# livesense-inc/fanlin-rs

Measured on AMD Instinct MI355X. Metric: images/sec whole-node (1080p→300×200 resize+encode); p50 per-image ms, higher is better.
Workload: dtype u8 (exact, as f16 subnormals) x the reference's f32 weights as three f16 terms -> f32 sums (vertical, v_mfma_f32_16x16x32_f16); 24-bit fixed-point intermediate (2^-14 steps, three i8 planes) x 24-bit fixed-point weights (2^-24 steps, three i8 digits), eight of the nine digit products -> exact i32 (h

## Files before the change

### fanlin-rs_amd/csrc/fl_jpeg_dev.h

```cpp
#pragma once
#include <hip/hip_runtime.h>
#include <stdint.h>

#include "fl_jpeg.h"
#include "fl_jpeg_tables.h"
#include "fl_pixel.h"
#include "fl_types.h"

namespace fl {

namespace {


constexpr int32_t F_0_298 = 2446, F_0_390 = 3196, F_0_541 = 4433, F_0_765 = 6270, F_0_899 = 7373, F_1_175 = 9633, F_1_501 = 12299,
                  F_1_847 = 15137, F_1_961 = 16069, F_2_053 = 16819, F_2_562 = 20995, F_3_072 = 25172;

struct Mat8 { int32_t a[8][8]; };

constexpr void fdct_linear(const int32_t in[8], int32_t out[8])
{
    int32_t t0 = in[0] + in[7], t1 = in[1] + in[6], t2 = in[2] + in[5], t3 = in[3] + in[4];
    const int32_t t10 = t0 + t3, t11 = t1 + t2;
    int32_t t12 = t0 - t3, t13 = t1 - t2;
    t0 = in[0] - in[7]; t1 = in[1] - in[6]; t2 = in[2] - in[5]; t3 = in[3] - in[4];
    out[0] = t10 + t11;
    out[4] = t10 - t11;
    int32_t z1 = (t12 + t13) * F_0_541;
    out[2] = z1 + t12 * F_0_765;
    out[6] = z1 - t13 * F_1_847;
    t12 = t0 + t2;
    t13 = t1 + t3;
    z1 = (t12 + t13) * F_1_175;
    t12 = t12 * (-F_0_390) + z1;
    t13 = t13 * (-F_1_961) + z1;
    z1 = (t0 + t3) * (-F_0_899);
    out[1] = t0 * F_1_501 + z1 + t12;
    out[7] = t3 * F_0_298 + z1 + t13;
    z1 = (t1 + t2) * (-F_2_562);
    out[3] = t1 * F_3_072 + z1 + t13;
    out[5] = t2 * F_2_053 + z1 + t12;
}

constexpr Mat8 make_fdct_matrix()
{
    Mat8 m{};
    for (int j = 0; j < 8; ++j) {
        int32_t e[8] = {0, 0, 0, 0, 0, 0, 0, 0}, o[8] = {0, 0, 0, 0, 0, 0, 0, 0};
        e[j] = 1;
        fdct_linear(e, o);
        for (int k = 0; k < 8; ++k) m.a[k][j] = o[k];
    }
    return m;
}

__constant__ Mat8 kFdct = make_fdct_matrix();

constexpr bool fdct_matrix_fits_i16()
{
    const Mat8 m = make_fdct_matrix();
    for (int k = 0; k < 8; ++k)
        for (int j = 0; j < 8; ++j)
            if (m.a[k][j] > 32767 || m.a[k][j] < -32768) return false;
    return true;
}
static_assert(fdct_matrix_fits_i16(), "the passes use v_dot2_i32_i16: matrix entries must be 16-bit");

typedef short i16x2 __attribute__((ext_vector_type(2)));
__device__ __forceinline__ i16x2 as_i16x2(uint32_t v) { return __builtin_bit_cast(i16x2, v); }
__device__ __forceinline__ uint32_t pack_i16(int32_t lo, int32_t hi) { return ((uint32_t)lo & 0xffffu) | ((uint32_t)hi << 16); }
__device__ __forceinline__ int32_t dot8_i16(const uint32_t m[4], const uint4 v)
{
    int32_t p = __builtin_amdgcn_sdot2(as_i16x2(m[0]), as_i16x2(v.x), 0, false);
    p = __builtin_amdgcn_sdot2(as_i16x2(m[1]), as_i16x2(v.y), p, false);
    p = __builtin_amdgcn_sdot2(as_i16x2(m[2]), as_i16x2(v.z), p, false);
    return __builtin_amdgcn_sdot2(as_i16x2(m[3]), as_i16x2(v.w), p, false);
}

struct NaturalOrder { uint8_t n[64]; };
constexpr NaturalOrder make_natural()
{
    NaturalOrder t{};
    for (int k = 0; k < 64; ++k) t.n[k] = kUnzigzag[k];
    return t;
}
__constant__ NaturalOrder kNatural = make_natural();

struct HuffLut { uint32_t e[256]; };

constexpr HuffLut make_lut(const HuffSpec &s)
{
    HuffLut t{};
    uint32_t code = 0;
    int k = 0;
    for (int l = 1; l <= 16; ++l) {
        for (int i = 0; i < s.len[l - 1]; ++i, ++k) t.e[s.val[k]] = ((uint32_t)l << 16) | code++;
        code <<= 1;
    }
    return t;
}

struct HuffAll { HuffLut ac[2], dc[2]; };
constexpr HuffAll make_all() { return HuffAll{{make_lut(kAcLuma), make_lut(kAcChroma)}, {make_lut(kDcLuma), make_lut(kDcChroma)}}; }
__constant__ HuffAll kHuff = make_all();


template <int N>
__device__ __forceinline__ uint32_t dpp_row_shr(uint32_t v)
{
    return (uint32_t)__builtin_amdgcn_update_dpp(0, (int)v, 0x110 + N, 0xf, 0xf, false);
}

__device__ __forceinline__ uint32_t wave_inclusive_scan(uint32_t v, uint32_t lane)
{
    (void)lane;
    v += dpp_row_shr<1>(v);
    v += dpp_row_shr<2>(v);
    v += dpp_row_shr<4>(v);
    v += dpp_row_shr<8>(v);
    v += (uint32_t)__builtin_amdgcn_update_dpp(0, (int)v, 0x142, 0xa, 0xf, false);
    v += (uint32_t)__builtin_amdgcn_update_dpp(0, (int)v, 0x143, 0xc, 0xf, false);
    return v;
}

__device__ __forceinline__ void wave_lds_sync()
{
    __builtin_amdgcn_fence(__ATOMIC_SEQ_CST, "wavefront");
    __builtin_amdgcn_wave_barrier();
}

constexpr uint32_t kPackThreads = 512;
constexpr uint32_t kPackWaves = kPackThreads / 64;

__device__ __forceinline__ uint32_t wg_exclusive_scan(uint32_t v, uint32_t *s_w, uint32_t *total)
{
    const uint32_t lane = threadIdx.x & 63u, wave = threadIdx.x >> 6;
    const uint32_t inc = wave_inclusive_scan(v, lane);
    __syncthreads();
    if (lane == 63u) s_w[wave] = inc;
    __syncthreads();
    uint32_t base = 0, sum = 0;
#pragma unroll
    for (uint32_t i = 0; i < kPackWaves; ++i) { const uint32_t t = s_w[i]; if (i < wave) base += t; sum += t; }
    *total = sum;
    return base + inc - v;
}

__device__ __forceinline__ uint32_t coef_size(int32_t v)
{
    const uint32_t mag = (uint32_t)(v < 0 ? -v : v);
    return mag ? 32u - (uint32_t)__clz(mag) : 0u;
}


#ifndef FL_JPEG_BPW
#define FL_JPEG_BPW 16
#define FL_JPEG_WPG 2
#define FL_JPEG_PREFETCH 3
#endif
constexpr uint32_t kBlocksPerWave = FL_JPEG_BPW;
constexpr uint32_t kWavesPerWg = FL_JPEG_WPG;
constexpr uint32_t kPrefetch = FL_JPEG_PREFETCH;
static_assert(kBlocksPerWave == 32u || kBlocksPerWave == 16u, "the coding phase's lane mapping");
constexpr uint32_t kJpegThreads = 64u * kWavesPerWg;
constexpr uint32_t kBlocksPerWg = kWavesPerWg * kBlocksPerWave;
constexpr uint32_t kUnitsPerWave = 3u * kBlocksPerWave;

static_assert(63u * (16u + 10u) <= kAcWordsPerUnit * 32u, "a unit's AC code must fit its acbits slot");

struct WaveLds {
    int16_t coef[kUnitsPerWave][64];
    uint64_t nz[kUnitsPerWave];
    __attribute__((aligned(16))) int16_t smp[3][64];
    __attribute__((aligned(16))) int16_t p1[3][64];
};

__device__ __forceinline__ void stage_ac_luts(uint32_t *s_ac, const uint32_t *own = nullptr)
{
    if (own) for (uint32_t i = threadIdx.x; i < 512u; i += kJpegThreads) s_ac[i] = own[i];
    else for (uint32_t i = threadIdx.x; i < 512u; i += kJpegThreads) s_ac[i] = kHuff.ac[i >> 8].e[i & 255u];
    __syncthreads();
}

template <bool kRgba>
__device__ __forceinline__ uint32_t block_pixel(const JpegJob &jb, uint32_t brow, uint32_t bcol, uint32_t r, uint32_t c)
{
    uint32_t px = bcol * 8u + c, py = brow * 8u + r;
    px = px < jb.w ? px : jb.w - 1u;
    py = py < jb.h ? py : jb.h - 1u;
    if constexpr (kRgba) return ((const __attribute__((address_space(1))) uint32_t *)jb.src)[(size_t)py * jb.w + px];
    uint32_t pr, pg, pb, pa;
    load_rgba(jb.src + ((size_t)py * jb.w + px) * jb.c, jb.c, pr, pg, pb, pa);
    return pr | (pg << 8) | (pb << 16);
}

__device__ __forceinline__ void dct_quant_block(const uint32_t (&smp)[3], uint32_t nat, uint32_t r, uint32_t c, const uint32_t (&m1)[4],
                                                const uint32_t (&m2)[4], uint4 k1, const uint32_t (&q)[3], const uint32_t (&magic)[3],
                                                WaveLds &w, int32_t (&qv)[3])
{
#pragma unroll
    for (int k = 0; k < 3; ++k) w.smp[k][nat] = (int16_t)smp[k];
    wave_lds_sync();
#pragma unroll
    for (int k = 0; k < 3; ++k) {
        const int32_t p = dot8_i16(m1, *reinterpret_cast<const uint4 *>(w.smp[k] + r * 8));
        const int32_t v1 = ((p << k1.x) + (int32_t)k1.y) >> 11;
        w.p1[k][c * 8 + r] = (int16_t)v1;
    }
    wave_lds_sync();
#pragma unroll
    for (int k = 0; k < 3; ++k) {
        const int32_t p2 = dot8_i16(m2, *reinterpret_cast<const uint4 *>(w.p1[k] + c * 8));
        const int32_t d = (p2 + (int32_t)k1.z) >> k1.w;
        const int32_t sg = d >> 31;
        const uint32_t an = (uint32_t)((d ^ sg) - sg) >> 3;
        const uint32_t rq = __umulhi(2u * an + q[k], magic[k]);
        qv[k] = ((int32_t)rq ^ sg) - sg;
    }
}

typedef __attribute__((address_space(1))) uint32_t global_u32;
typedef uint32_t u32x4 __attribute__((ext_vector_type(4)));
typedef __attribute__((address_space(1))) u32x4 global_u32x4;
static_assert(sizeof(JpegUnit) == sizeof(u32x4) && kUnitAcWords == 3u, "a unit's record is one 16-byte access");

struct UnitBits {
    uint64_t acc;
    uint32_t pend, total, wi;
    global_u32 *out;
    uint32_t w0, w1, w2;
    __device__ __forceinline__ void word(uint32_t v)
    {
        w0 = wi == 0u ? v : w0;
        w1 = wi == 1u ? v : w1;
        w2 = wi == 2u ? v : w2;
        if (wi >= kUnitAcWords) out[wi] = v;
        ++wi;
    }
    __device__ __forceinline__ void put(uint32_t code, uint32_t len)
    {
        acc = (acc << len) | code;
        pend += len;
        total += len;
        if (pend >= 32u) { pend -= 32u; word((uint32_t)(acc >> pend)); }
    }
};

template <bool kRgba>
__device__ __forceinline__ void transform_blocks(const JpegJob &jb, const uint32_t *__restrict__ arena, uint32_t first, uint32_t count,
                                                 uint32_t lane, WaveLds &w)
{
    const uint32_t nat = kNatural.n[lane], r = nat >> 3, c = nat & 7u;
    uint32_t m1[4], m2[4];
#pragma unroll
    for (int j = 0; j < 4; ++j) {
        m1[j] = pack_i16(kFdct.a[c][2 * j], kFdct.a[c][2 * j + 1]);
        m2[j] = pack_i16(kFdct.a[r][2 * j], kFdct.a[r][2 * j + 1]);
    }
    const uint8_t *qt = reinterpret_cast<const uint8_t *>(arena + jb.tab_off) + 624;
    const uint32_t *mg = reinterpret_cast<const uint32_t *>(qt + 128);
    const uint32_t q[3] = {qt[nat], qt[64 + nat], qt[64 + nat]};
    const uint32_t magic[3] = {mg[nat], mg[64 + nat], mg[64 + nat]};
    const uint4 k1 = {(c == 0u || c == 4u) ? 13u : 0u, c == 0u ? (uint32_t)(-(8 * 128) * 8192) : (c == 4u ? 0u : 1u << 10),
                      (r == 0u || r == 4u) ? 2u : 1u << 14, (r == 0u || r == 4u) ? 2u : 15u};
    uint32_t brow = first / jb.bx, bcol = first - brow * jb.bx;
    uint32_t ahead[kPrefetch];
#pragma unroll
    for (uint32_t j = 0; j < kPrefetch; ++j) {
        ahead[j] = block_pixel<kRgba>(jb, brow, bcol, r, c);
        if (++bcol == jb.bx) { bcol = 0; ++brow; }
    }
    for (uint32_t i = 0; i < count; ++i) {
        const uint32_t rgb = kRgba ? ahead[0] & 0xffffffu : ahead[0];
#pragma unroll
        for (uint32_t j = 0; j + 1u < kPrefetch; ++j) ahead[j] = ahead[j + 1u];
        ahead[kPrefetch - 1u] = block_pixel<kRgba>(jb, brow, bcol, r, c);
        if (++bcol == jb.bx) { bcol = 0; ++brow; }
        uint32_t smp[3];
        jfif_px(rgb, smp[0], smp[1], smp[2]);
        const bool flat = __ballot(rgb != (uint32_t)__builtin_amdgcn_readfirstlane((int)rgb)) == 0ull;
        if (flat) {
            if (lane == 0u) {
#pragma unroll
                for (int k = 0; k < 3; ++k) {
                    const int32_t d = 64 * ((int32_t)smp[k] - 128);
                    const int32_t sg = d >> 31;
                    const uint32_t an = (uint32_t)((d ^ sg) - sg) >> 3;
                    const uint32_t rq = __umulhi(2u * an + q[k], magic[k]);
                    w.coef[i * 3u + k][0] = (int16_t)(((int32_t)rq ^ sg) - sg);
                    w.nz[i * 3u + k] = 0ull;
                }
            }
            continue;
        }
        int32_t qv[3];
        dct_quant_block(smp, nat, r, c, m1, m2, k1, q, magic, w, qv);
#pragma unroll
        for (int k = 0; k < 3; ++k) {
            w.coef[i * 3u + k][lane] = (int16_t)qv[k];
            const uint64_t nz = __ballot(qv[k] != 0) & ~1ull;
            if (lane == 0u) w.nz[i * 3u + k] = nz;
        }
    }
}

template <bool kOwn>
__device__ __forceinline__ void jpeg_code_units(const JpegJob *__restrict__ jobs, const uint32_t *__restrict__ arena, uint32_t job_base,
                                                const uint32_t *__restrict__ opt)
{
    __shared__ WaveLds s_w[kWavesPerWg];
    __shared__ uint32_t s_ac[512];
    const JpegJob jb = jobs[job_base + blockIdx.y];
    const uint32_t wave = threadIdx.x >> 6, lane = threadIdx.x & 63u;
    const uint32_t nblocks = jb.bx * jb.by;
    if (blockIdx.x * kBlocksPerWg >= nblocks) return;
    if constexpr (kOwn) stage_ac_luts(s_ac, opt + jb.opt_off + kJpegOptAcLut);
    else stage_ac_luts(s_ac);
    const uint32_t first = blockIdx.x * kBlocksPerWg + wave * kBlocksPerWave;
    if (first >= nblocks) return;
    const uint32_t count = min(kBlocksPerWave, nblocks - first);
    WaveLds &w = s_w[wave];

    if (jb.c == 4u && (reinterpret_cast<uintptr_t>(jb.src) & 3u) == 0u) transform_blocks<true>(jb, arena, first, count, lane, w);
    else transform_blocks<false>(jb, arena, first, count, lane, w);
    wave_lds_sync();

    uint32_t b, u, u_end;
    bool chroma;
    if constexpr (kBlocksPerWave == 32u) {
        b = lane & 31u;
        chroma = lane >= 32u;
        u = b * 3u + (chroma ? 1u : 0u);
        u_end = b * 3u + (chroma ? 3u : 1u);
    } else {
        b = lane & 15u;
        chroma = lane >= 16u;
        u = b * 3u + (lane >> 4);
        u_end = lane >= 48u ? u : u + 1u;
    }
    if (b >= count) return;
    const uint32_t *tab = s_ac + (chroma ? 256u : 0u);
    const uint32_t eob = tab[0], zrl = tab[0xF0];
    for (; u < u_end; ++u) {
        const uint32_t unit = first * 3u + u;
        const int16_t *cf = w.coef[u];
        uint64_t m = w.nz[u];
        UnitBits ub{0ull, 0u, 0u, 0u, (global_u32 *)jb.acbits + (size_t)unit * kAcWordsPerUnit, 0u, 0u, 0u};
        uint32_t prev = 0;
        uint32_t pos = (uint32_t)__builtin_ctzll(m | (1ull << 63));
        int32_t v = cf[pos];
        while (m) {
            const uint32_t cpos = pos;
            const int32_t cv = v;
            m &= m - 1ull;
            pos = (uint32_t)__builtin_ctzll(m | (1ull << 63));
            v = cf[pos];
            uint32_t run = cpos - prev - 1u;
            prev = cpos;
            while (run > 15u) { ub.put(zrl & 0xffffu, zrl >> 16); run -= 16u; }
            const uint32_t mag = (uint32_t)(cv < 0 ? -cv : cv);
            const uint32_t size = 32u - (uint32_t)__clz(mag);
            const uint32_t value = (uint32_t)(cv + (cv >> 31)) & ((1u << size) - 1u);
            const uint32_t e = tab[(run << 4) | size];
            ub.put(((e & 0xffffu) << size) | value, (e >> 16) + size);
        }
        if (prev != 63u) ub.put(eob & 0xffffu, eob >> 16);
        if (ub.pend) ub.word((uint32_t)(ub.acc << (32u - ub.pend)));
        const u32x4 rec = {((uint32_t)(uint16_t)cf[0]) | (ub.total << 16), ub.w0, ub.w1, ub.w2};
        ((global_u32x4 *)jb.units)[unit] = rec;
    }
}


constexpr uint32_t kDcCodes = 12;

constexpr uint32_t kWinWords = 8192;

__device__ __forceinline__ void win_or(uint32_t *win, uint32_t wbase, uint64_t g, uint32_t val)
{
    const uint64_t W = g >> 5;
    const uint32_t sh = (uint32_t)g & 31u;
    const uint32_t hi = val >> sh, lo = sh ? val << (32u - sh) : 0u;
    if (hi && W >= wbase && W < (uint64_t)wbase + kWinWords) atomicOr(&win[W - wbase], hi);
    if (lo && W + 1 >= wbase && W + 1 < (uint64_t)wbase + kWinWords) atomicOr(&win[W + 1 - wbase], lo);
}

__device__ __forceinline__ uint32_t dc_code(const uint32_t *s_dc, uint32_t u, uint32_t meta, uint32_t prev_meta, uint32_t *len)
{
    const int32_t dc = (int16_t)(meta & 0xffffu), prev = (int16_t)(prev_meta & 0xffffu);
    const int32_t diff = dc - prev;
    const uint32_t size = coef_size(diff);
    const uint32_t value = (uint32_t)(diff < 0 ? diff - 1 : diff) & ((1u << size) - 1u);
    const uint32_t e = s_dc[((u % 3u) ? kDcCodes : 0u) + size];
    *len = (e >> 16) + size;
    return (((e & 0xffffu) << size) | value) << (32u - *len);
}

struct PackUnit { u32x4 rec; uint32_t prev; };
__device__ __forceinline__ PackUnit load_pack_unit(const JpegJob &jb, uint32_t u, uint32_t u_end)
{
    const global_u32x4 *recs = (const global_u32x4 *)jb.units;
    const uint32_t uc = min(u, u_end - 1u);
    PackUnit p;
    p.rec = recs[uc];
    p.prev = ((const global_u32 *)(recs + (max(uc, 3u) - 3u)))[0];
    return p;
}
__device__ __forceinline__ PackUnit take_pack_unit(PackUnit p, uint32_t u, uint32_t u_end)
{
    if (u >= u_end) p.rec = u32x4{0u, 0u, 0u, 0u};
    if (u < 3u || u >= u_end) p.prev = 0u;
    return p;
}

#ifndef FL_JPEG_PACK_DEPTH
#define FL_JPEG_PACK_DEPTH 1
#endif
constexpr uint32_t kPackDepth = FL_JPEG_PACK_DEPTH;

template <bool kOwn>
__global__ __launch_bounds__(kPackThreads) void jpeg_pack_kernel(const JpegJob *__restrict__ jobs, const uint32_t *__restrict__ arena,
                                                                 uint32_t job_base, const uint32_t *__restrict__ opt)
{
    __shared__ uint32_t s_win[kWinWords];
    __shared__ uint32_t s_w[kPackWaves], s_carry, s_lo, s_hi, s_dc[2u * kDcCodes];
    const JpegJob jb = jobs[job_base + blockIdx.x];
    const uint32_t tid = threadIdx.x;
    const uint32_t nunits = jb.bx * jb.by * 3u;
    constexpr uint32_t T = kPackThreads;

    PackUnit ahead[kPackDepth];
#pragma unroll
    for (uint32_t j = 0; j < kPackDepth; ++j) ahead[j] = load_pack_unit(jb, j * T + tid, nunits);
    for (uint32_t i = tid; i < kWinWords; i += T) s_win[i] = 0u;
    const uint32_t *own = kOwn ? opt + jb.opt_off : nullptr;
    if constexpr (kOwn) { if (tid < 2u * kDcCodes) s_dc[tid] = own[kJpegOptDcLut + tid]; }
    else if (tid < 2u * kDcCodes) s_dc[tid] = kHuff.dc[tid / kDcCodes].e[tid % kDcCodes];
    if (tid == 0u) s_carry = 0u;
    __syncthreads();
    for (uint32_t base0 = 0; base0 < nunits; base0 += kPackDepth * T) {
#pragma unroll
        for (uint32_t j = 0; j < kPackDepth; ++j) {
            const uint32_t base = base0 + j * T;
            if (base >= nunits) break;
            const uint32_t u = base + tid;
            const PackUnit next = load_pack_unit(jb, u + kPackDepth * T, nunits);
            const PackUnit cur = take_pack_unit(ahead[j], u, nunits);
            ahead[j] = next;
            const uint32_t m = cur.rec.x;
            const uint32_t nw = ((m >> 16) + 31u) >> 5;
            uint32_t len = 0, dl = 0, dcw = 0;
            if (u < nunits) {
                dcw = dc_code(s_dc, u, m, cur.prev, &dl);
                len = dl + (m >> 16);
            }
            uint32_t chunk;
            const uint32_t ex = wg_exclusive_scan(len, s_w, &chunk);
            const uint32_t carry = s_carry;
            if (u < nunits) {
                const uint32_t off = carry + ex;
                ((global_u32 *)jb.unit_off)[u] = off;
                win_or(s_win, 0u, off, dcw);
                win_or(s_win, 0u, (uint64_t)off + dl, cur.rec.y);
                win_or(s_win, 0u, (uint64_t)off + dl + 32u, cur.rec.z);
                win_or(s_win, 0u, (uint64_t)off + dl + 64u, cur.rec.w);
                for (uint32_t w = kUnitAcWords; w < nw; ++w)
                    win_or(s_win, 0u, (uint64_t)off + dl + 32u * w, ((const global_u32 *)jb.acbits)[(size_t)u * kAcWordsPerUnit + w]);
            }
            __syncthreads();
            if (tid == 0u) s_carry = carry + chunk;
            __syncthreads();
        }
    }
    const uint32_t total_bits = s_carry;
    if (tid == 0u) jb.unit_off[nunits] = total_bits;
    __threadfence_block();
    __syncthreads();
    const uint32_t nbytes = (total_bits + 7u) >> 3, limit = jb.dst_cap;
    const uint8_t *hdr = reinterpret_cast<const uint8_t *>(kOwn ? own + kJpegOptHeader : arena + jb.tab_off);
    const uint32_t hdr_bytes = kOwn ? own[kJpegOptHdrLen] : kJpegHeaderBytes;
    for (uint32_t i = tid; i < hdr_bytes; i += T) if (i < limit) jb.dst[i] = hdr[i];

    uint32_t ff_before = 0;
    for (uint32_t wbase = 0; wbase * 32ull < total_bits; wbase += kWinWords) {
        const uint64_t wb = (uint64_t)wbase * 32u, we = wb + (uint64_t)kWinWords * 32u;
        if (wbase != 0u) {
            for (uint32_t i = tid; i < kWinWords; i += T) s_win[i] = 0u;
            if (tid == 0u) {
                uint32_t lo = 0, hi = nunits;
                while (lo < hi) { const uint32_t mid = (lo + hi) >> 1; if (jb.unit_off[mid + 1u] > wb) hi = mid; else lo = mid + 1u; }
                s_lo = lo;
                uint32_t lo2 = lo, hi2 = nunits;
                while (lo2 < hi2) { const uint32_t mid = (lo2 + hi2) >> 1; if (jb.unit_off[mid] >= we) hi2 = mid; else lo2 = mid + 1u; }
                s_hi = lo2;
            }
        } else if (tid == 0u) { s_lo = 0u; s_hi = 0u; }
        __syncthreads();
        const uint32_t u_lo = s_lo, u_hi = s_hi;
        for (uint32_t ub = u_lo; ub < u_hi; ub += T / 2u) {
            const uint32_t u = ub + (tid >> 1), j = tid & 1u;
            if (u < u_hi) {
                const PackUnit p = take_pack_unit(load_pack_unit(jb, u, u_hi), u, u_hi);
                const uint32_t m = p.rec.x, off = jb.unit_off[u];
                uint32_t dl;
                const uint32_t dcw = dc_code(s_dc, u, m, p.prev, &dl);
                if (j == 0u) win_or(s_win, wbase, off, dcw);
                const uint32_t nw = ((m >> 16) + 31u) >> 5;
                win_or(s_win, wbase, (uint64_t)off + dl + 32u * j, j ? p.rec.z : p.rec.y);
                if (j == 0u) win_or(s_win, wbase, (uint64_t)off + dl + 64u, p.rec.w);
                for (uint32_t w = j ? 3u : 4u; w < nw; w += 2u)
                    win_or(s_win, wbase, (uint64_t)off + dl + 32u * w, ((const global_u32 *)jb.acbits)[(size_t)u * kAcWordsPerUnit + w]);
            }
        }
        __syncthreads();
        if (tid == 0u && (total_bits & 7u) && (total_bits >> 5) >= wbase && (total_bits >> 5) < wbase + kWinWords)
            s_win[(total_bits >> 5) - wbase] |= (0xFFu >> (total_bits & 7u)) << (24u - 8u * ((total_bits >> 3) & 3u));
        __syncthreads();
        const uint32_t win_bytes = (uint32_t)min((uint64_t)kWinWords * 4u, (uint64_t)nbytes - (uint64_t)wbase * 4u);
        if (tid == 0u) s_carry = 0u;
        __syncthreads();
        for (uint32_t base = 0; base < win_bytes; base += 4u * T) {
            const uint32_t i = base + tid * 4u;
            const uint32_t word = i < win_bytes ? s_win[i >> 2] : 0u;
            const uint32_t valid = i < win_bytes ? (win_bytes - i < 4u ? win_bytes - i : 4u) : 0u;
            uint32_t ff = 0;
#pragma unroll
            for (uint32_t k = 0; k < 4; ++k) ff += (k < valid && ((word >> (24u - 8u * k)) & 255u) == 255u) ? 1u : 0u;
            uint32_t chunk;
            const uint32_t ex = wg_exclusive_scan(ff, s_w, &chunk);
            const uint32_t carry = s_carry;
            uint64_t o = (uint64_t)hdr_bytes + (uint64_t)wbase * 4u + i + ff_before + carry + ex;
#pragma unroll
            for (uint32_t k = 0; k < 4; ++k) {
                if (k < valid) {
                    const uint32_t b = (word >> (24u - 8u * k)) & 255u;
                    if (o < limit) jb.dst[o] = (uint8_t)b;
                    ++o;
                    if (b == 255u) { if (o < limit) jb.dst[o] = 0u; ++o; }
                }
            }
            __syncthreads();
            if (tid == 0u) s_carry = carry + chunk;
            __syncthreads();
        }
        ff_before += s_carry;
        __syncthreads();
    }
    if (tid == 0u) {
        const uint64_t end = (uint64_t)hdr_bytes + nbytes + ff_before;
        if (end + 2u <= limit) {
            jb.dst[end] = 0xFF; jb.dst[end + 1u] = 0xD9;
            jb.result[1] = (uint32_t)(end + 2u);
            if constexpr (kOwn) { if (own[kJpegOptFlag]) atomicOr(&jb.result[0], FL_JPEG_RESULT_OPTIMIZED); }
        } else {
            jb.result[1] = 0u;
            atomicOr(&jb.result[0], FL_JPEG_RESULT_OVERFLOW);
        }
    }
}

}

}
```

### fanlin-rs_amd/csrc/fl_jpeg_opt.hip

```cpp
#include "fl_jpeg_dev.h"
#include "fl_jpeg_opt_core.h"

namespace fl {

namespace {

__global__ __launch_bounds__(kJpegThreads) void jpeg_opt_code_kernel(const JpegJob *__restrict__ jobs, const uint32_t *__restrict__ arena,
                                                                     uint32_t job_base, const uint32_t *__restrict__ opt)
{
    jpeg_code_units<true>(jobs, arena, job_base, opt);
}

__global__ __launch_bounds__(kJpegThreads) void jpeg_opt_stats_kernel(const JpegJob *__restrict__ jobs, const uint32_t *__restrict__ arena,
                                                                      uint32_t job_base, uint32_t *__restrict__ opt, uint32_t *__restrict__ hist)
{
    __shared__ WaveLds s_w[kWavesPerWg];
    __shared__ uint32_t s_hist[kJpegOptHistWords];
    const JpegJob jb = jobs[job_base + blockIdx.y];
    const uint32_t wave = threadIdx.x >> 6, lane = threadIdx.x & 63u;
    const uint32_t nblocks = jb.bx * jb.by;
    if (blockIdx.x * kBlocksPerWg >= nblocks) return;
    for (uint32_t i = threadIdx.x; i < kJpegOptHistWords; i += kJpegThreads) s_hist[i] = 0u;
    __syncthreads();
    const uint32_t first = blockIdx.x * kBlocksPerWg + wave * kBlocksPerWave;
    if (first < nblocks) {
        const uint32_t count = min(kBlocksPerWave, nblocks - first);
        WaveLds &w = s_w[wave];
        if (jb.c == 4u && (reinterpret_cast<uintptr_t>(jb.src) & 3u) == 0u) transform_blocks<true>(jb, arena, first, count, lane, w);
        else transform_blocks<false>(jb, arena, first, count, lane, w);
        wave_lds_sync();
        uint32_t b, u, u_end;
        bool chroma;
        if constexpr (kBlocksPerWave == 32u) {
            b = lane & 31u;
            chroma = lane >= 32u;
            u = b * 3u + (chroma ? 1u : 0u);
            u_end = b * 3u + (chroma ? 3u : 1u);
        } else {
            b = lane & 15u;
            chroma = lane >= 16u;
            u = b * 3u + (lane >> 4);
            u_end = lane >= 48u ? u : u + 1u;
        }
        if (b >= count) u_end = u;
        uint32_t *h = s_hist + (chroma ? 256u : 0u);
        int16_t *dcs = reinterpret_cast<int16_t *>(opt + jb.opt_off + kJpegOptHeadWords);
        for (; u < u_end; ++u) {
            const int16_t *cf = w.coef[u];
            uint64_t m = w.nz[u];
            dcs[first * 3u + u] = cf[0];
            uint32_t prev = 0;
            while (m) {
                const uint32_t pos = (uint32_t)__builtin_ctzll(m);
                m &= m - 1ull;
                const int32_t cv = cf[pos];
                uint32_t run = pos - prev - 1u;
                prev = pos;
                while (run > 15u) { atomicAdd(&h[0xF0], 1u); run -= 16u; }
                const uint32_t mag = (uint32_t)(cv < 0 ? -cv : cv);
                atomicAdd(&h[(run << 4) | (32u - (uint32_t)__clz(mag))], 1u);
            }
            if (prev != 63u) atomicAdd(&h[0], 1u);
        }
    }
    __syncthreads();
    uint32_t *g = hist + (size_t)blockIdx.y * kJpegOptHistWords;
    for (uint32_t i = threadIdx.x; i < kJpegOptHistWords; i += kJpegThreads) {
        const uint32_t v = s_hist[i];
        if (v) atomicAdd(&g[i], v);
    }
}

constexpr uint32_t kOptThreads = 256;

__device__ __forceinline__ uint32_t std_lut(uint32_t t, uint32_t s) { return (t & 1u) ? kHuff.ac[t >> 1].e[s] : kHuff.dc[t >> 1].e[s]; }

__global__ __launch_bounds__(kOptThreads) void jpeg_opt_tables_kernel(const JpegJob *__restrict__ jobs, const uint32_t *__restrict__ arena,
                                                                      uint32_t job_base, uint32_t *__restrict__ opt,
                                                                      const uint32_t *__restrict__ hist, uint32_t fallback)
{
    __shared__ uint32_t s_cnt[4][256];
    __shared__ uint32_t s_A[4][kJpegOptMaxLeaves + 1u];
    __shared__ JpegOptCode s_code[4];
    __shared__ uint8_t s_len[4][256], s_vals[4][256];
    __shared__ unsigned long long s_bits[3];
    __shared__ uint32_t s_used[4];
    const JpegJob jb = jobs[job_base + blockIdx.x];
    const uint32_t tid = threadIdx.x, nunits = jb.bx * jb.by * 3u;
    uint32_t *rec = opt + jb.opt_off;
    const uint32_t *g = hist + (size_t)blockIdx.x * kJpegOptHistWords;
    s_cnt[0][tid] = 0u; s_cnt[2][tid] = 0u;
    s_cnt[1][tid] = g[tid]; s_cnt[3][tid] = g[256u + tid];
    if (tid < 3u) s_bits[tid] = 0ull;
    __syncthreads();
    const int16_t *dcs = reinterpret_cast<const int16_t *>(rec + kJpegOptHeadWords);
    for (uint32_t u = tid; u < nunits; u += kOptThreads) {
        const int32_t diff = (int32_t)dcs[u] - (u >= 3u ? (int32_t)dcs[u - 3u] : 0);
        atomicAdd(&s_cnt[(u % 3u) ? 2u : 0u][coef_size(diff)], 1u);
    }
    __syncthreads();
    uint32_t rank[4];
#pragma unroll
    for (uint32_t t = 0; t < 4u; ++t) {
        uint32_t used;
        rank[t] = jpeg_opt_rank(s_cnt[t], tid, &used);
        if (s_cnt[t][tid]) s_A[t][1u + rank[t]] = s_cnt[t][tid];
        if (tid == 0u) { s_used[t] = used; s_A[t][0] = 1u; }
    }
    __syncthreads();
    if ((tid & 63u) == 0u) jpeg_opt_lengths(s_A[tid >> 6], (int)s_used[tid >> 6] + 1, s_code[tid >> 6]);
    __syncthreads();
#pragma unroll
    for (uint32_t t = 0; t < 4u; ++t) s_len[t][tid] = s_cnt[t][tid] ? (uint8_t)jpeg_opt_length_of_rank(s_code[t].num, rank[t]) : (uint8_t)0;
    __syncthreads();
    uint32_t lut[4];
    unsigned long long own = 0, std_bits = 0, val = 0;
#pragma unroll
    for (uint32_t t = 0; t < 4u; ++t) {
        const uint32_t l = s_len[t][tid], n = s_cnt[t][tid];
        lut[t] = 0u;
        if (l) {
            const uint32_t pos = jpeg_opt_pos(s_len[t], tid);
            lut[t] = (l << 16) | (s_code[t].first_code[l] + pos);
            s_vals[t][s_code[t].first_idx[l] + pos] = (uint8_t)tid;
            own += (unsigned long long)n * l;
            std_bits += (unsigned long long)n * (std_lut(t, tid) >> 16);
            val += (unsigned long long)n * jpeg_opt_value_bits(t, tid);
        }
    }
    if (own) { atomicAdd(&s_bits[0], own); atomicAdd(&s_bits[1], std_bits); }
    if (val) atomicAdd(&s_bits[2], val);
    __syncthreads();
    const uint32_t used[4] = {s_used[0], s_used[1], s_used[2], s_used[3]};
    const uint32_t own_header = jpeg_opt_header_bytes(used);
    const bool on = jpeg_opt_decide(own_header, s_bits[0], s_bits[1], s_bits[2], fallback != 0u);
    if (tid == 0u) { rec[kJpegOptHdrLen] = on ? own_header : kJpegHeaderBytes; rec[kJpegOptFlag] = on ? 1u : 0u; }
    if (tid < kDcCodes) {
        rec[kJpegOptDcLut + tid] = on ? lut[0] : std_lut(0, tid);
        rec[kJpegOptDcLut + kDcCodes + tid] = on ? lut[2] : std_lut(2, tid);
    }
    rec[kJpegOptAcLut + tid] = on ? lut[1] : std_lut(1, tid);
    rec[kJpegOptAcLut + 256u + tid] = on ? lut[3] : std_lut(3, tid);
    const uint8_t *hdr = reinterpret_cast<const uint8_t *>(arena + jb.tab_off);
    uint8_t *out = reinterpret_cast<uint8_t *>(rec + kJpegOptHeader);
    if (!on) {
        for (uint32_t i = tid; i < kJpegHeaderBytes; i += kOptThreads) out[i] = hdr[i];
        return;
    }
    if (tid < kJpegOptPrefixBytes) out[tid] = hdr[tid];
    uint32_t at = kJpegOptPrefixBytes;
#pragma unroll
    for (uint32_t t = 0; t < 4u; ++t) {
        if (tid < kJpegOptDhtHead) out[at + tid] = jpeg_opt_dht_head(t, tid, s_code[t].num, used[t]);
        if (tid < used[t]) out[at + kJpegOptDhtHead + tid] = s_vals[t][tid];
        at += kJpegOptDhtHead + used[t];
    }
    if (tid < kJpegOptSosBytes) out[at + tid] = hdr[kJpegHeaderBytes - kJpegOptSosBytes + tid];
}

}

hipError_t launch_jpeg_encode_optimized(const JpegJob *jobs, const uint32_t *arena, uint32_t job_base, uint32_t njobs, uint32_t max_blocks,
                                        uint32_t *opt, uint32_t *hist, bool fallback, hipStream_t st)
{
    if (!njobs || !max_blocks) return hipSuccess;
    const dim3 grid((max_blocks + kBlocksPerWg - 1) / kBlocksPerWg, njobs);
    if (hipError_t e = hipMemsetAsync(hist, 0, (size_t)njobs * kJpegOptHistWords * sizeof(uint32_t), st)) return e;
    hipLaunchKernelGGL(jpeg_opt_stats_kernel, grid, dim3(kJpegThreads), 0, st, jobs, arena, job_base, opt, hist);
    FL_LAUNCH_CHECK();
    hipLaunchKernelGGL(jpeg_opt_tables_kernel, dim3(njobs), dim3(kOptThreads), 0, st, jobs, arena, job_base, opt, (const uint32_t *)hist, fallback ? 1u : 0u);
    FL_LAUNCH_CHECK();
    hipLaunchKernelGGL(jpeg_opt_code_kernel, grid, dim3(kJpegThreads), 0, st, jobs, arena, job_base, (const uint32_t *)opt);
    FL_LAUNCH_CHECK();
    hipLaunchKernelGGL(jpeg_pack_kernel<true>, dim3(njobs), dim3(kPackThreads), 0, st, jobs, arena, job_base, (const uint32_t *)opt);
    FL_LAUNCH_CHECK();
    return hipSuccess;
}

}
```

Before: 577,800.

## Keep per-unit nonzero masks in registers and streamline DCT/quant arithmetic

Replaces the LDS nonzero-mask array with per-lane registers filled via writelane, so the coding phase reads its mask without touching shared memory. Folds the row-pass scaling into the DCT matrix so pass-1 rounding becomes a dot-product start value, and switches quantisation to 24-bit multiply intrinsics. Replaces per-pixel clamp arithmetic with an incremental block walker whose interior blocks use a precomputed offset, and unrolls the prefetch ring into named slots. The 32-blocks-per-wave configuration is dropped, and the u24 quantiser changes the magic-number precision, which risks off-by-one quantised values.

```diff
diff --git a/fanlin-rs_amd/csrc/fl_jpeg_dev.h b/fanlin-rs_amd/csrc/fl_jpeg_dev.h
--- a/fanlin-rs_amd/csrc/fl_jpeg_dev.h
+++ b/fanlin-rs_amd/csrc/fl_jpeg_dev.h
@@ -6,6 +6,10 @@
 #include "fl_jpeg_tables.h"
 #include "fl_pixel.h"
 #include "fl_types.h"
+
+extern "C" __device__ int fl_writelane_i32(int value, int lane, int old) __asm("llvm.amdgcn.writelane.i32");
+extern "C" __device__ uint32_t fl_mul_u24(uint32_t a, uint32_t b) __asm("llvm.amdgcn.mul.u24.i32");
+extern "C" __device__ uint32_t fl_mulhi_u24(uint32_t a, uint32_t b) __asm("llvm.amdgcn.mulhi.u24");
 
 namespace fl {
 
@@ -53,24 +57,46 @@
     return m;
 }
 
-__constant__ Mat8 kFdct = make_fdct_matrix();
-
-constexpr bool fdct_matrix_fits_i16()
-{
-    const Mat8 m = make_fdct_matrix();
+constexpr int32_t kRowScale = 8192;
+constexpr Mat8 make_pass_matrix()
+{
+    Mat8 m = make_fdct_matrix();
+    for (int j = 0; j < 8; ++j) { m.a[0][j] *= kRowScale; m.a[4][j] *= kRowScale; }
+    return m;
+}
+
+__constant__ Mat8 kFdct = make_pass_matrix();
+
+constexpr bool pass_matrix_fits_i16()
+{
+    const Mat8 m = make_pass_matrix();
     for (int k = 0; k < 8; ++k)
         for (int j = 0; j < 8; ++j)
             if (m.a[k][j] > 32767 || m.a[k][j] < -32768) return false;
     return true;
 }
-static_assert(fdct_matrix_fits_i16(), "the passes use v_dot2_i32_i16: matrix entries must be 16-bit");
+static_assert(pass_matrix_fits_i16(), "the passes use v_dot2_i32_i16: matrix entries must be 16-bit");
+
+constexpr int64_t pass_matrix_bound(int64_t in_max)
+{
+    const Mat8 m = make_pass_matrix();
+    int64_t worst = 0;
+    for (int k = 0; k < 8; ++k) {
+        int64_t sum = 0;
+        for (int j = 0; j < 8; ++j) sum += (m.a[k][j] < 0 ? -(int64_t)m.a[k][j] : (int64_t)m.a[k][j]) * in_max;
+        worst = sum > worst ? sum : worst;
+    }
+    return worst;
+}
+static_assert(pass_matrix_bound(255) <= 2040ll * kRowScale && 2040ll * kRowScale + 1024ll * kRowScale < (1ll << 31), "pass 1 stays in 32 bits");
+static_assert(pass_matrix_bound(8160) <= 65280ll * kRowScale && 65280ll * kRowScale + (1ll << 14) < (1ll << 31), "pass 2 stays in 32 bits");
 
 typedef short i16x2 __attribute__((ext_vector_type(2)));
 __device__ __forceinline__ i16x2 as_i16x2(uint32_t v) { return __builtin_bit_cast(i16x2, v); }
 __device__ __forceinline__ uint32_t pack_i16(int32_t lo, int32_t hi) { return ((uint32_t)lo & 0xffffu) | ((uint32_t)hi << 16); }
-__device__ __forceinline__ int32_t dot8_i16(const uint32_t m[4], const uint4 v)
-{
-    int32_t p = __builtin_amdgcn_sdot2(as_i16x2(m[0]), as_i16x2(v.x), 0, false);
+__device__ __forceinline__ int32_t dot8_i16(const uint32_t m[4], const uint4 v, int32_t start)
+{
+    int32_t p = __builtin_amdgcn_sdot2(as_i16x2(m[0]), as_i16x2(v.x), start, false);
     p = __builtin_amdgcn_sdot2(as_i16x2(m[1]), as_i16x2(v.y), p, false);
     p = __builtin_amdgcn_sdot2(as_i16x2(m[2]), as_i16x2(v.z), p, false);
     return __builtin_amdgcn_sdot2(as_i16x2(m[3]), as_i16x2(v.w), p, false);
@@ -152,15 +178,9 @@
 }
 
 
-#ifndef FL_JPEG_BPW
-#define FL_JPEG_BPW 16
-#define FL_JPEG_WPG 2
-#define FL_JPEG_PREFETCH 3
-#endif
-constexpr uint32_t kBlocksPerWave = FL_JPEG_BPW;
-constexpr uint32_t kWavesPerWg = FL_JPEG_WPG;
-constexpr uint32_t kPrefetch = FL_JPEG_PREFETCH;
-static_assert(kBlocksPerWave == 32u || kBlocksPerWave == 16u, "the coding phase's lane mapping");
+constexpr uint32_t kBlocksPerWave = 16;
+constexpr uint32_t kWavesPerWg = 2;
+constexpr uint32_t kPrefetch = 3;
 constexpr uint32_t kJpegThreads = 64u * kWavesPerWg;
 constexpr uint32_t kBlocksPerWg = kWavesPerWg * kBlocksPerWave;
 constexpr uint32_t kUnitsPerWave = 3u * kBlocksPerWave;
@@ -169,7 +189,6 @@
 
 struct WaveLds {
     int16_t coef[kUnitsPerWave][64];
-    uint64_t nz[kUnitsPerWave];
     __attribute__((aligned(16))) int16_t smp[3][64];
     __attribute__((aligned(16))) int16_t p1[3][64];
 };
@@ -181,44 +200,88 @@
     __syncthreads();
 }
 
+typedef __attribute__((address_space(1))) uint32_t global_u32;
+typedef __attribute__((address_space(1))) uint8_t global_u8;
+
+struct BlockWalk {
+    uint32_t brow, bcol, rlim, clim;
+    const global_u8 *origin;
+    __device__ __forceinline__ void row(const JpegJob &jb)
+    {
+        const uint32_t b = min(brow, jb.by - 1u);
+        rlim = jb.h - 1u - b * 8u;
+        clim = jb.w - 1u;
+        origin = (const global_u8 *)jb.src + (size_t)b * 8u * jb.w * 4u;
+    }
+    __device__ __forceinline__ void start(const JpegJob &jb, uint32_t first)
+    {
+        brow = first / jb.bx;
+        bcol = first - brow * jb.bx;
+        row(jb);
+        clim -= bcol * 8u;
+        origin += bcol * 32u;
+    }
+    __device__ __forceinline__ void next(const JpegJob &jb)
+    {
+        clim -= 8u;
+        origin += 32u;
+        if (++bcol == jb.bx) { bcol = 0; ++brow; row(jb); }
+    }
+};
+
 template <bool kRgba>
-__device__ __forceinline__ uint32_t block_pixel(const JpegJob &jb, uint32_t brow, uint32_t bcol, uint32_t r, uint32_t c)
-{
-    uint32_t px = bcol * 8u + c, py = brow * 8u + r;
+__device__ __forceinline__ uint32_t block_pixel(const JpegJob &jb, const BlockWalk &bw, uint32_t r, uint32_t c, uint32_t inner)
+{
+    if constexpr (kRgba) {
+        uint32_t off = inner;
+        if (bw.rlim < 7u || bw.clim < 7u) off = (min(r, bw.rlim) * jb.w + min(c, bw.clim)) * 4u;
+        return *(const global_u32 *)(bw.origin + off);
+    }
+    uint32_t px = bw.bcol * 8u + c, py = bw.brow * 8u + r;
     px = px < jb.w ? px : jb.w - 1u;
     py = py < jb.h ? py : jb.h - 1u;
-    if constexpr (kRgba) return ((const __attribute__((address_space(1))) uint32_t *)jb.src)[(size_t)py * jb.w + px];
     uint32_t pr, pg, pb, pa;
     load_rgba(jb.src + ((size_t)py * jb.w + px) * jb.c, jb.c, pr, pg, pb, pa);
     return pr | (pg << 8) | (pb << 16);
 }
 
+struct Quantiser { uint32_t q8, m24; };
+__device__ __forceinline__ Quantiser make_quantiser(uint32_t q, uint32_t magic32) { return Quantiser{q << 8, (magic32 + 255u) >> 8}; }
+__device__ __forceinline__ int32_t quantise_magnitude(uint32_t an, int32_t sg, const Quantiser &z)
+{
+    const uint32_t x = fl_mul_u24(an, 512u) + z.q8;
+    const uint32_t rq = fl_mulhi_u24(x, z.m24);
+    return ((int32_t)rq ^ sg) - sg;
+}
+__device__ __forceinline__ int32_t quantise(int32_t d, const Quantiser &z)
+{
+    const int32_t sg = d >> 31;
+    return quantise_magnitude((uint32_t)((d ^ sg) - sg) >> 3, sg, z);
+}
+__device__ __forceinline__ int32_t quantise_sum15(int32_t sum, const Quantiser &z)
+{
+    const int32_t sg = sum >> 31;
+    return quantise_magnitude((uint32_t)((sum ^ sg) + (sg & 0x8000)) >> 18, sg, z);
+}
+
 __device__ __forceinline__ void dct_quant_block(const uint32_t (&smp)[3], uint32_t nat, uint32_t r, uint32_t c, const uint32_t (&m1)[4],
-                                                const uint32_t (&m2)[4], uint4 k1, const uint32_t (&q)[3], const uint32_t (&magic)[3],
-                                                WaveLds &w, int32_t (&qv)[3])
+                                                const uint32_t (&m2)[4], int32_t k1, const Quantiser (&z)[3], WaveLds &w, int32_t (&qv)[3])
 {
 #pragma unroll
     for (int k = 0; k < 3; ++k) w.smp[k][nat] = (int16_t)smp[k];
     wave_lds_sync();
 #pragma unroll
     for (int k = 0; k < 3; ++k) {
-        const int32_t p = dot8_i16(m1, *reinterpret_cast<const uint4 *>(w.smp[k] + r * 8));
-        const int32_t v1 = ((p << k1.x) + (int32_t)k1.y) >> 11;
+        const int32_t v1 = dot8_i16(m1, *reinterpret_cast<const uint4 *>(w.smp[k] + r * 8), k1) >> 11;
         w.p1[k][c * 8 + r] = (int16_t)v1;
     }
     wave_lds_sync();
 #pragma unroll
     for (int k = 0; k < 3; ++k) {
-        const int32_t p2 = dot8_i16(m2, *reinterpret_cast<const uint4 *>(w.p1[k] + c * 8));
-        const int32_t d = (p2 + (int32_t)k1.z) >> k1.w;
-        const int32_t sg = d >> 31;
-        const uint32_t an = (uint32_t)((d ^ sg) - sg) >> 3;
-        const uint32_t rq = __umulhi(2u * an + q[k], magic[k]);
-        qv[k] = ((int32_t)rq ^ sg) - sg;
-    }
-}
-
-typedef __attribute__((address_space(1))) uint32_t global_u32;
+        qv[k] = quantise_sum15(dot8_i16(m2, *reinterpret_cast<const uint4 *>(w.p1[k] + c * 8), 1 << 14), z[k]);
+    }
+}
+
 typedef uint32_t u32x4 __attribute__((ext_vector_type(4)));
 typedef __attribute__((address_space(1))) u32x4 global_u32x4;
 static_assert(sizeof(JpegUnit) == sizeof(u32x4) && kUnitAcWords == 3u, "a unit's record is one 16-byte access");
@@ -245,9 +308,19 @@
     }
 };
 
+struct UnitMask {
+    uint32_t lo, hi;
+    __device__ __forceinline__ void set(uint32_t lane_of_unit, uint64_t m)
+    {
+        lo = (uint32_t)fl_writelane_i32((int)(uint32_t)m, (int)lane_of_unit, (int)lo);
+        hi = (uint32_t)fl_writelane_i32((int)(uint32_t)(m >> 32), (int)lane_of_unit, (int)hi);
+    }
+    __device__ __forceinline__ uint64_t bits() const { return ((uint64_t)hi << 32) | lo; }
+};
+
 template <bool kRgba>
-__device__ __forceinline__ void transform_blocks(const JpegJob &jb, const uint32_t *__restrict__ arena, uint32_t first, uint32_t count,
-                                                 uint32_t lane, WaveLds &w)
+__device__ __forceinline__ UnitMask transform_blocks(const JpegJob &jb, const uint32_t *__restrict__ arena, uint32_t first, uint32_t count,
+                                                     uint32_t lane, WaveLds &w)
 {
     const uint32_t nat = kNatural.n[lane], r = nat >> 3, c = nat & 7u;
     uint32_t m1[4], m2[4];
@@ -258,49 +331,65 @@
     }
     const uint8_t *qt = reinterpret_cast<const uint8_t *>(arena + jb.tab_off) + 624;
     const uint32_t *mg = reinterpret_cast<const uint32_t *>(qt + 128);
-    const uint32_t q[3] = {qt[nat], qt[64 + nat], qt[64 + nat]};
-    const uint32_t magic[3] = {mg[nat], mg[64 + nat], mg[64 + nat]};
-    const uint4 k1 = {(c == 0u || c == 4u) ? 13u : 0u, c == 0u ? (uint32_t)(-(8 * 128) * 8192) : (c == 4u ? 0u : 1u << 10),
-                      (r == 0u || r == 4u) ? 2u : 1u << 14, (r == 0u || r == 4u) ? 2u : 15u};
-    uint32_t brow = first / jb.bx, bcol = first - brow * jb.bx;
-    uint32_t ahead[kPrefetch];
-#pragma unroll
-    for (uint32_t j = 0; j < kPrefetch; ++j) {
-        ahead[j] = block_pixel<kRgba>(jb, brow, bcol, r, c);
-        if (++bcol == jb.bx) { bcol = 0; ++brow; }
-    }
-    for (uint32_t i = 0; i < count; ++i) {
-        const uint32_t rgb = kRgba ? ahead[0] & 0xffffffu : ahead[0];
-#pragma unroll
-        for (uint32_t j = 0; j + 1u < kPrefetch; ++j) ahead[j] = ahead[j + 1u];
-        ahead[kPrefetch - 1u] = block_pixel<kRgba>(jb, brow, bcol, r, c);
-        if (++bcol == jb.bx) { bcol = 0; ++brow; }
+    const Quantiser z[3] = {make_quantiser(qt[nat], mg[nat]), make_quantiser(qt[64 + nat], mg[64 + nat]), make_quantiser(qt[64 + nat], mg[64 + nat])};
+    const int32_t k1 = c == 0u ? -(8 * 128) * kRowScale : (c == 4u ? 0 : 1 << 10);
+    const uint32_t inner = (r * jb.w + c) * 4u;
+    UnitMask mask{0u, 0u};
+    BlockWalk bw;
+    bw.start(jb, first);
+    static_assert(kPrefetch == 3u, "the ring's slots are named");
+    auto ahead = [&] { const uint32_t px = block_pixel<kRgba>(jb, bw, r, c, inner); bw.next(jb); return px; };
+    uint32_t slot0 = ahead();
+    uint32_t slot1 = ahead();
+    uint32_t slot2 = ahead();
+    auto block = [&](uint32_t i, uint32_t &slot) {
+        uint32_t rgb = kRgba ? slot & 0xffffffu : slot;
+        asm volatile("" : "+v"(rgb));
+        slot = ahead();
         uint32_t smp[3];
         jfif_px(rgb, smp[0], smp[1], smp[2]);
         const bool flat = __ballot(rgb != (uint32_t)__builtin_amdgcn_readfirstlane((int)rgb)) == 0ull;
         if (flat) {
             if (lane == 0u) {
 #pragma unroll
-                for (int k = 0; k < 3; ++k) {
-                    const int32_t d = 64 * ((int32_t)smp[k] - 128);
-                    const int32_t sg = d >> 31;
-                    const uint32_t an = (uint32_t)((d ^ sg) - sg) >> 3;
-                    const uint32_t rq = __umulhi(2u * an + q[k], magic[k]);
-                    w.coef[i * 3u + k][0] = (int16_t)(((int32_t)rq ^ sg) - sg);
-                    w.nz[i * 3u + k] = 0ull;
-                }
+                for (int k = 0; k < 3; ++k) w.coef[i * 3u + k][0] = (int16_t)quantise(64 * ((int32_t)smp[k] - 128), z[k]);
             }
-            continue;
+            return;
         }
         int32_t qv[3];
-        dct_quant_block(smp, nat, r, c, m1, m2, k1, q, magic, w, qv);
+        dct_quant_block(smp, nat, r, c, m1, m2, k1, z, w, qv);
 #pragma unroll
         for (int k = 0; k < 3; ++k) {
             w.coef[i * 3u + k][lane] = (int16_t)qv[k];
-            const uint64_t nz = __ballot(qv[k] != 0) & ~1ull;
-            if (lane == 0u) w.nz[i * 3u + k] = nz;
+            mask.set(16u * k + i, __ballot(qv[k] != 0) & ~1ull);
         }
-    }
+    };
+    for (uint32_t i = 0;;) {
+        block(i, slot0);
+        if (++i == count) break;
+        block(i, slot1);
+        if (++i == count) break;
+        block(i, slot2);
+        if (++i == count) break;
+    }
+    return mask;
+}
+
+struct WaveBlocks { uint32_t wave, first, count; };
+__device__ __forceinline__ WaveBlocks wave_blocks(uint32_t nblocks)
+{
+    WaveBlocks b;
+    b.wave = (uint32_t)__builtin_amdgcn_readfirstlane((int)(threadIdx.x >> 6));
+    b.first = blockIdx.x * kBlocksPerWg + b.wave * kBlocksPerWave;
+    b.count = b.first < nblocks ? min(kBlocksPerWave, nblocks - b.first) : 0u;
+    return b;
+}
+
+__device__ __forceinline__ UnitMask transform_wave(const JpegJob &jb, const uint32_t *__restrict__ arena, const WaveBlocks &wb, uint32_t lane,
+                                                   WaveLds &w)
+{
+    if (jb.c == 4u && (reinterpret_cast<uintptr_t>(jb.src) & 3u) == 0u) return transform_blocks<true>(jb, arena, wb.first, wb.count, lane, w);
+    return transform_blocks<false>(jb, arena, wb.first, wb.count, lane, w);
 }
 
 template <bool kOwn>
@@ -310,64 +399,48 @@
     __shared__ WaveLds s_w[kWavesPerWg];
     __shared__ uint32_t s_ac[512];
     const JpegJob jb = jobs[job_base + blockIdx.y];
-    const uint32_t wave = threadIdx.x >> 6, lane = threadIdx.x & 63u;
+    const uint32_t lane = threadIdx.x & 63u;
     const uint32_t nblocks = jb.bx * jb.by;
     if (blockIdx.x * kBlocksPerWg >= nblocks) return;
     if constexpr (kOwn) stage_ac_luts(s_ac, opt + jb.opt_off + kJpegOptAcLut);
     else stage_ac_luts(s_ac);
-    const uint32_t first = blockIdx.x * kBlocksPerWg + wave * kBlocksPerWave;
-    if (first >= nblocks) return;
-    const uint32_t count = min(kBlocksPerWave, nblocks - first);
-    WaveLds &w = s_w[wave];
-
-    if (jb.c == 4u && (reinterpret_cast<uintptr_t>(jb.src) & 3u) == 0u) transform_blocks<true>(jb, arena, first, count, lane, w);
-    else transform_blocks<false>(jb, arena, first, count, lane, w);
+    const WaveBlocks wb = wave_blocks(nblocks);
+    if (!wb.count) return;
+    WaveLds &w = s_w[wb.wave];
+
+    const UnitMask mask = transform_wave(jb, arena, wb, lane, w);
     wave_lds_sync();
 
-    uint32_t b, u, u_end;
-    bool chroma;
-    if constexpr (kBlocksPerWave == 32u) {
-        b = lane & 31u;
-        chroma = lane >= 32u;
-        u = b * 3u + (chroma ? 1u : 0u);
-        u_end = b * 3u + (chroma ? 3u : 1u);
-    } else {
-        b = lane & 15u;
-        chroma = lane >= 16u;
-        u = b * 3u + (lane >> 4);
-        u_end = lane >= 48u ? u : u + 1u;
-    }
-    if (b >= count) return;
-    const uint32_t *tab = s_ac + (chroma ? 256u : 0u);
+    const uint32_t b = lane & 15u, u = b * 3u + (lane >> 4);
+    if (b >= wb.count || lane >= 48u) return;
+    const uint32_t *tab = s_ac + (lane >= 16u ? 256u : 0u);
     const uint32_t eob = tab[0], zrl = tab[0xF0];
-    for (; u < u_end; ++u) {
-        const uint32_t unit = first * 3u + u;
-        const int16_t *cf = w.coef[u];
-        uint64_t m = w.nz[u];
-        UnitBits ub{0ull, 0u, 0u, 0u, (global_u32 *)jb.acbits + (size_t)unit * kAcWordsPerUnit, 0u, 0u, 0u};
-        uint32_t prev = 0;
-        uint32_t pos = (uint32_t)__builtin_ctzll(m | (1ull << 63));
-        int32_t v = cf[pos];
-        while (m) {
-            const uint32_t cpos = pos;
-            const int32_t cv = v;
-            m &= m - 1ull;
-            pos = (uint32_t)__builtin_ctzll(m | (1ull << 63));
-            v = cf[pos];
-            uint32_t run = cpos - prev - 1u;
-            prev = cpos;
-            while (run > 15u) { ub.put(zrl & 0xffffu, zrl >> 16); run -= 16u; }
-            const uint32_t mag = (uint32_t)(cv < 0 ? -cv : cv);
-            const uint32_t size = 32u - (uint32_t)__clz(mag);
-            const uint32_t value = (uint32_t)(cv + (cv >> 31)) & ((1u << size) - 1u);
-            const uint32_t e = tab[(run << 4) | size];
-            ub.put(((e & 0xffffu) << size) | value, (e >> 16) + size);
-        }
-        if (prev != 63u) ub.put(eob & 0xffffu, eob >> 16);
-        if (ub.pend) ub.word((uint32_t)(ub.acc << (32u - ub.pend)));
-        const u32x4 rec = {((uint32_t)(uint16_t)cf[0]) | (ub.total << 16), ub.w0, ub.w1, ub.w2};
-        ((global_u32x4 *)jb.units)[unit] = rec;
-    }
+    const uint32_t unit = wb.first * 3u + u;
+    const int16_t *cf = w.coef[u];
+    uint64_t m = mask.bits();
+    UnitBits ub{0ull, 0u, 0u, 0u, (global_u32 *)jb.acbits + (size_t)unit * kAcWordsPerUnit, 0u, 0u, 0u};
+    uint32_t prev = 0;
+    uint32_t pos = (uint32_t)__builtin_ctzll(m | (1ull << 63));
+    int32_t v = cf[pos];
+    while (m) {
+        const uint32_t cpos = pos;
+        const int32_t cv = v;
+        m &= m - 1ull;
+        pos = (uint32_t)__builtin_ctzll(m | (1ull << 63));
+        v = cf[pos];
+        uint32_t run = cpos - prev - 1u;
+        prev = cpos;
+        while (run > 15u) { ub.put(zrl & 0xffffu, zrl >> 16); run -= 16u; }
+        const uint32_t mag = (uint32_t)(cv < 0 ? -cv : cv);
+        const uint32_t size = 32u - (uint32_t)__clz(mag);
+        const uint32_t value = (uint32_t)(cv + (cv >> 31)) & ((1u << size) - 1u);
+        const uint32_t e = tab[(run << 4) | size];
+        ub.put(((e & 0xffffu) << size) | value, (e >> 16) + size);
+    }
+    if (prev != 63u) ub.put(eob & 0xffffu, eob >> 16);
+    if (ub.pend) ub.word((uint32_t)(ub.acc << (32u - ub.pend)));
+    const u32x4 rec = {((uint32_t)(uint16_t)cf[0]) | (ub.total << 16), ub.w0, ub.w1, ub.w2};
+    ((global_u32x4 *)jb.units)[unit] = rec;
 }
 
 
diff --git a/fanlin-rs_amd/csrc/fl_jpeg_opt.hip b/fanlin-rs_amd/csrc/fl_jpeg_opt.hip
--- a/fanlin-rs_amd/csrc/fl_jpeg_opt.hip
+++ b/fanlin-rs_amd/csrc/fl_jpeg_opt.hip
@@ -17,38 +17,23 @@
     __shared__ WaveLds s_w[kWavesPerWg];
     __shared__ uint32_t s_hist[kJpegOptHistWords];
     const JpegJob jb = jobs[job_base + blockIdx.y];
-    const uint32_t wave = threadIdx.x >> 6, lane = threadIdx.x & 63u;
+    const uint32_t lane = threadIdx.x & 63u;
     const uint32_t nblocks = jb.bx * jb.by;
     if (blockIdx.x * kBlocksPerWg >= nblocks) return;
     for (uint32_t i = threadIdx.x; i < kJpegOptHistWords; i += kJpegThreads) s_hist[i] = 0u;
     __syncthreads();
-    const uint32_t first = blockIdx.x * kBlocksPerWg + wave * kBlocksPerWave;
-    if (first < nblocks) {
-        const uint32_t count = min(kBlocksPerWave, nblocks - first);
-        WaveLds &w = s_w[wave];
-        if (jb.c == 4u && (reinterpret_cast<uintptr_t>(jb.src) & 3u) == 0u) transform_blocks<true>(jb, arena, first, count, lane, w);
-        else transform_blocks<false>(jb, arena, first, count, lane, w);
+    const WaveBlocks wb = wave_blocks(nblocks);
+    if (wb.count) {
+        WaveLds &w = s_w[wb.wave];
+        const UnitMask mask = transform_wave(jb, arena, wb, lane, w);
         wave_lds_sync();
-        uint32_t b, u, u_end;
-        bool chroma;
-        if constexpr (kBlocksPerWave == 32u) {
-            b = lane & 31u;
-            chroma = lane >= 32u;
-            u = b * 3u + (chroma ? 1u : 0u);
-            u_end = b * 3u + (chroma ? 3u : 1u);
-        } else {
-            b = lane & 15u;
-            chroma = lane >= 16u;
-            u = b * 3u + (lane >> 4);
-            u_end = lane >= 48u ? u : u + 1u;
-        }
-        if (b >= count) u_end = u;
-        uint32_t *h = s_hist + (chroma ? 256u : 0u);
+        const uint32_t b = lane & 15u, u = b * 3u + (lane >> 4);
+        uint32_t *h = s_hist + (lane >= 16u ? 256u : 0u);
         int16_t *dcs = reinterpret_cast<int16_t *>(opt + jb.opt_off + kJpegOptHeadWords);
-        for (; u < u_end; ++u) {
+        if (b < wb.count && lane < 48u) {
             const int16_t *cf = w.coef[u];
-            uint64_t m = w.nz[u];
-            dcs[first * 3u + u] = cf[0];
+            uint64_t m = mask.bits();
+            dcs[wb.first * 3u + u] = cf[0];
             uint32_t prev = 0;
             while (m) {
                 const uint32_t pos = (uint32_t)__builtin_ctzll(m);
```

New measurement: 569,300. 1.5% lower.
